# Zoe187419/ATE_replication_causalML

Hardware: AMD Instinct MI355X
Metric: rows/sec for DML-ATE cross-fit, N=1e7 p=500, 1/2/4/8 MI355X; ATE/SE parity (higher is better)
Workload: dtype bf16; 1 GPU; model=DML-PLR 5-fold cross-fit, CV-LASSO nuisances (100 lambdas, inner 4-fold CV), global_batch=10000000, seq_len=500, N=10000000, p=500, folds=5, parallelism=dp1, dgp=tutorial, n_kept=10000000, layout=blocked64+bytes8

## Files before the change

### ate_replication_causalml_amd/_native.py

```python
from __future__ import annotations

import ctypes
import os
from pathlib import Path

_LIBDIR = Path(__file__).resolve().parent / "_lib"
_hip = None
_cpu = None


class NativeMissing(RuntimeError):
    pass


class NativeError(RuntimeError):

    def __init__(self, name: str, status: int, detail: str):
        self.entry, self.status = name, status
        super().__init__(f"{name} failed with status {status}: {detail}")


HIP_ERRORS = {
    1: "hipErrorInvalidValue", 2: "hipErrorOutOfMemory", 3: "hipErrorNotInitialized",
    4: "hipErrorDeinitialized", 9: "hipErrorInvalidConfiguration",
# ... 37 lines not shown
    "ate_chol_solve": "pipiipdpppppp",
    "ate_chol_solve_k": "pipipidppppp",
    "ate_spd_solve_batched": "ppiippp",
    "ate_predict": "ipllppiidipp",
    "ate_irls_update": "ipllppiiiiippppipp",
    "ate_irls_check": "piidippp",
    "ate_naive": "ippplpppp",
    "ate_clip_propensity": "pplpp",
    "ate_aipw": "ppppppldpppp",
    "ate_dml_moments": "ppplppp",
    "ate_dml_finalize": "pipp",
    "ate_boot_multinomial": "ppluiipp",
    "ate_boot_poisson": "ppluiilipp",
    "ate_enet_prepare": "piipipiipipipppppppp",
    "ate_enet_prepare_fused": "piipipiipipi" + "ppppppp" + "plp",
    "ate_enet_path": "pipiippppidddipppppippp",
    "ate_enet_coef": "ppiiiipppppppp",
    "ate_enet_cvloss_gauss": "pippiipppiiipp",
    "ate_cv_select": "pppiipippppip",
    "ate_enet_pick": "ppiiipppip",
    "ate_enet_cv_tail": "pippiipppi" + "pppppp" + "iiii" + "pppppppppppp",
    "ate_dml_resid_moments": "ipllpipipiiiiiippp",
    "ate_dml_resid_moments_final": "ipllpipipiiiiii" + "ppppp",
    "ate_dml_resid_exact": "pllpipipiiiiiiippp",
    "ate_irm_score_moments": "ipllpipiipiiiiidippp",
    "ate_irm_score_moments_multi": "ipllpipiipipiiiiiidippp",
    "ate_irm_score_multi_smax": "",
    "ate_irm_scores": "ipllpipiipiiiiidipp",
    "ate_irm_sens_moments": "ipllpipiipiiiiidippp",
    "ate_irm_target_moments": "ipllpipiipiiiiidippp",
# ... 170 lines not shown
```

### ate_replication_causalml_amd/estimators/lasso.py

```python
from __future__ import annotations

import numpy as np
import torch

from .. import _native
from ..ops import enet as enet_ops
from ..ops import stats as S
from ..ops.devconst import const
from ..ops.enet import cv_enet_gaussian
from ..ops.gram import gram
from ..ops.linalg import chol_solve, chol_solve_active
from ..ops.panel import build_panel, dtype_code
from ..parallel import rng
from ..reference.estimators import lambda_interp
from ..result import AteResult
from ..utils.graphs import estimator_graphs
from .common import as_np, read_result, resolve_device


def _fold_ids(n, K, seed, stream, dist):
    return dist.fold_ids(K, seed, stream) if dist is not None else rng.fold_ids(n, K, seed, stream)


def _sharded_gram(pan, dist):
# ... 306 lines not shown
            return None
        cv = cv_enet_gaussian(st["G"], pan, pan.xcols, ycols,
                              full_sets=[full_sets[k] for k in mine], seg_counts=seg_counts)
        return cv

    def pick(cv):
        return (cv.coef_min if lambda_rule == "min" else cv.coef_1se).reshape(
            len(mine), 2, -1).contiguous()

    fused_final = enet_ops.CV_FUSED and not dist and pan.data.is_cuda

    def phase_fit(st):
        cv = fit(st)
        coef = pick(cv)
        if fused_final:
            mom, res = dml_residual_moments(pan, coef, final=True)
            return {**st, "cv": cv, "mom": mom, "res": res}
        return {**st, "cv": cv, "mom": dml_residual_moments(pan, coef)}

    def phase_fit_sharded(st):
        cv = fit(st)
        coef = torch.zeros((K, 2, p1), dtype=torch.float64, device=pan.device)
        if cv is not None:
            coef.index_copy_(0, const(mine, torch.int64, pan.device), pick(cv).double())
        return {**st, "cv": cv, "coef": coef}

    def phase_resid(st):
        return {**st, "mom": dml_residual_moments(pan, st["coef"])}

    def phase_final(st):
        if "res" in st:
# ... 163 lines not shown
    dev = pan.device
    xc = const(pan.xcols, torch.int32, dev)
    segs = const(np.asarray(pan.seg_bounds[:K], dtype=np.int64), torch.int64, dev)
    nbx = 512
    part = torch.empty(K * nbx * (7 if mode == 1 else 14), dtype=torch.float64, device=dev)
    cs, bs = pan.strides()
    c = coef.double().contiguous()
    _native.call("ate_dml_resid_exact", pan.data.data_ptr(), cs, bs, xc.data_ptr(), len(pan.xcols),
                 segs.data_ptr(), K, c.data_ptr(), pan.cols["Y_hi"], pan.cols["Y_lo"],
                 pan.cols["W_hi"], pan.cols["W_lo"], pan.cols["one"], nbx, mode,
                 None if sh is None else sh.data_ptr(), part.data_ptr(),
                 torch.cuda.current_stream().cuda_stream)
    return part


def dml_residual_moments(pan, coef: torch.Tensor, final: bool = False):
    K = coef.shape[0]
    p = len(pan.xcols)
    if not pan.data.is_cuda:
        X = pan.colmajor().double()
        moms = torch.zeros(7, dtype=torch.float64)
        for k in range(K):
            r0, r1 = pan.seg_bounds[k]
            Xs = X[:, r0:r1]
            v = Xs[pan.cols["one"]] != 0
            xs = Xs[pan.xcols]
            yv, wv = Xs[pan.cols["Y"]], Xs[pan.cols["W"]]
            yr = yv - (coef[k, 0, 0] + coef[k, 0, 1:] @ xs)
            wr = wv - (coef[k, 1, 0] + coef[k, 1, 1:] @ xs)
            moms += S.dml_moments(yr[v], wr[v])
        return moms
    dev = pan.device
    xc = const(pan.xcols, torch.int32, dev)
    segs = const(np.asarray(pan.seg_bounds[:K], dtype=np.int64), torch.int64, dev)
    bf = pan.dtype == torch.bfloat16
    nbx = 512 if bf else 256
    part = torch.empty(K * nbx * 7, dtype=torch.float64, device=dev)
    mom = torch.empty(7, dtype=torch.float64, device=dev)
    bf = pan.dtype == torch.bfloat16
    y0, y1 = (pan.cols["Y_hi"], pan.cols["Y_lo"]) if bf else (pan.cols["Y"], -1)
    w0, w1 = (pan.cols["W_hi"], pan.cols["W_lo"]) if bf else (pan.cols["W"], -1)
    cs, bs = pan.strides()
    if final:
        res = torch.empty(2, dtype=torch.float64, device=dev)
        done = torch.zeros(1, dtype=torch.int32, device=dev)
        _native.call("ate_dml_resid_moments_final", dtype_code(pan.data), pan.data.data_ptr(), cs,
                     bs, xc.data_ptr(), p, segs.data_ptr(), K, coef.data_ptr(), y0, y1, w0, w1,
                     pan.cols["one"], nbx, part.data_ptr(), done.data_ptr(), mom.data_ptr(),
                     res.data_ptr(), torch.cuda.current_stream().cuda_stream)
        return mom, res
    _native.call("ate_dml_resid_moments", dtype_code(pan.data), pan.data.data_ptr(), cs, bs,
                 xc.data_ptr(), p, segs.data_ptr(), K, coef.data_ptr(), y0, y1, w0, w1,
                 pan.cols["one"], nbx, part.data_ptr(), mom.data_ptr(),
                 torch.cuda.current_stream().cuda_stream)
    return mom


def _dml_body(pan, folds, lambda_rule, dist=None, counts=None):
    comm = dist.comm if dist is not None else None
    return dml_crossfit_panel(pan, folds, lambda_rule, comm=comm,
# ... 48 lines not shown
```

### ate_replication_causalml_amd/ops/enet.py

```python
from __future__ import annotations

import os
from dataclasses import dataclass

import numpy as np
import torch

from .. import _native
from ..reference import glmnet as ref
from .devconst import const, const_bytes


def _stream():
    return torch.cuda.current_stream().cuda_stream


CV_FUSED = os.environ.get("ATE_CV_FUSED", "1") not in ("", "0")


@dataclass
class EnetCvResult:
    lambdas: torch.Tensor
    nlam: torch.Tensor
    cvm: torch.Tensor
    cvsd: torch.Tensor
    sel: torch.Tensor
    coef_path: torch.Tensor
    coef_min: torch.Tensor
    coef_1se: torch.Tensor
    full_keys: list
    npass: torch.Tensor
    fold_npass: torch.Tensor | None = None
    fold_nlam: torch.Tensor | None = None

    def check(self):
        bad = [] if self.fold_npass is None else \
            np.flatnonzero(self.fold_npass.cpu().numpy() < 0).tolist()
        if bad:
            from ..utils.guards import NumericalError
            raise NumericalError(f"CV fold path(s) {bad} timed out waiting for their "
                                 "full-data lambda sequence; selection is invalid")
        return self


def poison_if_truncated(fold_npass: torch.Tensor, *ts):
    bad = (fold_npass < 0).any()
    nan = torch.full((), float("nan"), dtype=torch.float64, device=fold_npass.device)
    return [torch.where(bad, nan, t) for t in ts]


def _zeroed(dev, *specs):
    sizes = [int(np.prod(sh)) * torch.empty((), dtype=dt).element_size() for sh, dt in specs]
    offs = np.concatenate([[0], np.cumsum([(b + 255) // 256 * 256 for b in sizes])])
    buf = torch.zeros(int(offs[-1]), dtype=torch.uint8, device=dev)
    return [buf[int(o):int(o) + b].view(dt).view(sh)
            for (sh, dt), o, b in zip(specs, offs[:-1], sizes)]


def _rescale_vp(vp, p):
    vp = np.ones(p) if vp is None else np.maximum(np.asarray(vp, float), 0)
    return vp * p / vp.sum()


def _cv_tables(nseg, full_sets, ycols, nreal, nlambda, full_y):
    ny = len(ycols)
    if full_sets is None:
        full_sets = [list(range(nseg))]
    tsets, tindex = [], {}

    def tid(segs):
        key = tuple(sorted(segs))
# ... 97 lines not shown
    nt = masks.shape[0]
    masks_t = const(masks, torch.uint8, dev)
    xc = const(xcols, torch.int32, dev)
    yc = const(ycols, torch.int32, dev)
    c_f32 = int(panel_dtype != torch.float64)
    ldc = (p + 63) // 64 * 64
    nf = len(full_probs)
    probs_all = list(full_probs) + list(fold_probs)
    nq = len(probs_all)
    i32 = torch.int32
    c_dt = torch.float32 if c_f32 else torch.float64
    fused = CV_FUSED and L <= 256
    fused_prep = fused and nseg <= 8
    if fused:
        zspec = [((nq, L), torch.float64), ((nq,), i32), ((nq,), i32), ((nq,), i32), ((nf,), i32)]
        if not fused_prep:
            zspec.append(((nt, p, ldc), c_dt))
        rsq, nlam, npass, progress, done, *zc = _zeroed(dev, *zspec)
        C = zc[0] if zc else torch.empty((nt, p, ldc), dtype=c_dt, device=dev)
        apath = torch.empty((nq, L, p), **f64)
    else:
        C, apath, rsq, nlam, npass, progress = _zeroed(
            dev, ((nt, p, ldc), c_dt), ((nq, L, p), torch.float64),
            ((nq, L), torch.float64), ((nq,), i32), ((nq,), i32), ((nq,), i32))
    g = torch.empty((nt, ny, p), **f64)
    xm = torch.empty((nt, p), **f64)
    xs = torch.empty((nt, p), **f64)
    ju = torch.empty((nt, p), dtype=torch.uint8, device=dev)
    ym = torch.empty((nt, ny), **f64)
    ys = torch.empty((nt, ny), **f64)
    nobs = torch.empty(nt, **f64)
    if fused_prep:
        lams = torch.empty((nq, L), **f64)
        _native.call("ate_enet_prepare_fused", G.data_ptr(), nseg, P, masks_t.data_ptr(), nt,
                     xc.data_ptr(), p, one, yc.data_ptr(), ny, C.data_ptr(), c_f32, g.data_ptr(),
                     xm.data_ptr(), xs.data_ptr(), ju.data_ptr(), ym.data_ptr(), ys.data_ptr(),
                     nobs.data_ptr(), lams.data_ptr(), nq * L, s)
    else:
        _native.call("ate_enet_prepare", G.data_ptr(), nseg, P, masks_t.data_ptr(), nt,
                     xc.data_ptr(), p, one, yc.data_ptr(), ny, C.data_ptr(), c_f32, g.data_ptr(),
                     xm.data_ptr(), xs.data_ptr(), ju.data_ptr(), ym.data_ptr(), ys.data_ptr(),
                     nobs.data_ptr(), s)
        lams = torch.full((nq, L), float("nan"), **f64)
    vp_t = const(np.asarray(vp, dtype=np.float64), torch.float64, dev)
    pr = _probs_tensor(probs_all, dev)
    lampub = torch.empty((nq, L), **f64)
    _native.call("ate_enet_path", C.data_ptr(), c_f32, g.data_ptr(), p, ny, ju.data_ptr(),
                 ys.data_ptr(), vp_t.data_ptr(), pr.data_ptr(), nq, alpha, flmin, thresh,
                 maxit, apath.data_ptr(), lams.data_ptr(), rsq.data_ptr(), nlam.data_ptr(),
                 npass.data_ptr(), L, progress.data_ptr(), lampub.data_ptr(), s)
    hold = const([0] * nf + list(fold_holds), torch.int32, dev)
    ycol_p = const([0] * nf + list(fold_ycol), torch.int32, dev)
# ... 4 lines not shown
    cvsd = torch.empty((nf, L), **f64)
    sel = torch.empty((nf, 2), dtype=torch.int32, device=dev)
    K = fold_index.shape[1]
    cmin = torch.empty((nf, p + 1), **f64)
    c1se = torch.empty((nf, p + 1), **f64)
    fold_npass = npass[nf:]
    if fused:
        coef = torch.empty((nf, L, p + 1), **f64)
        _native.call("ate_enet_cv_tail", G.data_ptr(), P, hold.data_ptr(), xc.data_ptr(), p, one,
                     ycol_p.data_ptr(), apath.data_ptr(), pr.data_ptr(), ny, nlam.data_ptr(),
                     xm.data_ptr(), xs.data_ptr(), ju.data_ptr(), ym.data_ptr(), ys.data_ptr(), L,
                     nf, nq - nf, K, fidx.data_ptr(), nfold_t.data_ptr(), coef.data_ptr(),
                     cvraw.data_ptr(), cvm.data_ptr(), cvsd.data_ptr(), sel.data_ptr(),
                     cmin.data_ptr(), c1se.data_ptr(), fold_npass.data_ptr(), done.data_ptr(), s)
        return EnetCvResult(lams[:nf], nlam[:nf], cvm, cvsd, sel, coef, cmin, c1se, full_keys,
                            npass[:nf], fold_npass, nlam[nf:])
    coef = torch.empty((nq, L, p + 1), **f64)
    _native.call("ate_enet_coef", apath.data_ptr(), pr.data_ptr(), nq, p, ny, L,
                 nlam.data_ptr(), xm.data_ptr(), xs.data_ptr(), ju.data_ptr(), ym.data_ptr(),
                 ys.data_ptr(), coef.data_ptr(), s)
    _native.call("ate_enet_cvloss_gauss", G.data_ptr(), P, hold.data_ptr(), xc.data_ptr(), p, one,
                 ycol_p.data_ptr(), coef.data_ptr(), nlam.data_ptr(), L, nf, nq - nf,
                 cvraw.data_ptr(), s)
    _native.call("ate_cv_select", cvraw.data_ptr(), fidx.data_ptr(), nfold_t.data_ptr(), K, nf,
                 nlam.data_ptr(), L, cvm.data_ptr(), cvsd.data_ptr(), sel.data_ptr(),
                 fold_npass.data_ptr(), nq - nf, s)
    _native.call("ate_enet_pick", coef.data_ptr(), sel.data_ptr(), p, L, nf, cmin.data_ptr(),
                 c1se.data_ptr(), fold_npass.data_ptr(), nq - nf, s)
    return EnetCvResult(lams[:nf], nlam[:nf], cvm, cvsd, sel, coef[:nf], cmin, c1se, full_keys,
                        npass[:nf], fold_npass, nlam[nf:])

# ... 79 lines not shown
```

### csrc/enet.hip

```cpp
#include <cstdlib>

#include <utility>

#include "common.hpp"

#include <type_traits>

using namespace ate;

__device__ __forceinline__ double seg_sum(const double* __restrict__ G, int nseg, int P,
                                          const unsigned char* __restrict__ mk, int a, int b) {
  double acc = 0.0;
  for (int q = 0; q < nseg; ++q)
    if (mk[q]) acc += G[((int64_t)q * P + a) * P + b];
  return acc;
}

__device__ __forceinline__ void col_mean_var(double s1, double s2, double n, double& m,
                                             double& v) {
  m = s1 / n;
  v = s2 / n - m * m;
}
__device__ __forceinline__ double std_entry(double sab, double n, double ma, double mb,
                                            double sa, double sb) {
// ... 106 lines not shown
  for (int q = 0; q < PF_SEG; ++q) v[q] = q < nseg ? G[((int64_t)q * P + a) * P + b] : 0.0;
  double acc = 0.0;
#pragma unroll
  for (int q = 0; q < PF_SEG; ++q)
    if (q < nseg && (bits >> q & 1u)) acc += v[q];
  return acc;
}

template <typename CT>
__global__ __launch_bounds__(256) void enet_prepare_fused_kernel(
    const double* __restrict__ G, int nseg, int P, const unsigned char* __restrict__ masks,
    int ntrain, const int* __restrict__ xcols, int p, int ldc, int ones_col,
    const int* __restrict__ ycols, int ny, CT* __restrict__ C, double* __restrict__ g,
    double* __restrict__ xm, double* __restrict__ xs, unsigned char* __restrict__ ju,
    double* __restrict__ ym, double* __restrict__ ys, double* __restrict__ nobs,
    double* __restrict__ lams, int64_t nlams) {
  const int tk = blockIdx.x, tj = blockIdx.y, tid = threadIdx.x;
  const int j0 = tj * PF_TJ, k0 = tk * PF_TK, s0 = blockIdx.z * PF_SCH;
  const int lane = tid & 63, jr = tid >> 6;
  ATE_DASSERT(k0 + PF_TK <= ldc && j0 < p && ones_col >= 0 && ones_col < P);
  {
    const int64_t nb = (int64_t)gridDim.x * gridDim.y * gridDim.z,
                  b = ((int64_t)blockIdx.z * gridDim.y + tj) * gridDim.x + tk;
    for (int64_t e = b * 256 + tid; e < nlams; e += nb * 256) lams[e] = __builtin_nan("");
  }
  __shared__ double s_n[PF_SCH], s_m[PF_SCH][PF_NC], s_s[PF_SCH][PF_NC];
  __shared__ unsigned char s_ju[PF_SCH][PF_NC];
  __shared__ unsigned s_mask[PF_SCH];
  const bool inreg = nseg <= PF_SEG;
  const int k = k0 + lane;
  const int xk = k < p ? xcols[k] : 0;
  ATE_DASSERT(xk >= 0 && xk < P);
  double gv[4][PF_SEG];
  int xj[4];
#pragma unroll
  for (int i = 0; i < 4; ++i) {
    const int j = j0 + jr + 4 * i;
    xj[i] = j < p ? xcols[j] : 0;
    ATE_DASSERT(xj[i] >= 0 && xj[i] < P);
// ... 87 lines not shown
        double gj = 0.0;
        if (s_ju[sl][jl]) {
          const int yc = ycols[y];
          ATE_DASSERT(yc >= 0 && yc < P);
          double my, vy;
          col_mean_var(set_sum(s, sl, ones_col, yc), set_sum(s, sl, yc, yc), s_n[sl], my, vy);
          gj = std_entry(set_sum(s, sl, xcols[j], yc), s_n[sl], s_m[sl][jl], my, s_s[sl][jl],
                         vy > 0 ? sqrt(vy) : 1.0);
        }
        g[((int64_t)s * ny + y) * p + j] = gj;
      }
    }
  }
}

ATE_API int ate_enet_prepare_fused(const void* G, int nseg, int P, const void* masks, int ntrain,
                                   const void* xcols, int p, int ones_col, const void* ycols,
                                   int ny, void* C, int c_f32, void* g, void* xm, void* xs,
                                   void* ju, void* ym, void* ys, void* nobs, void* lams,
                                   int64_t nlams, void* stream) {
  if (p < 1 || ntrain < 1 || nseg < 1 || ny < 0) return -1;
  hipStream_t st = (hipStream_t)stream;
  const int ldc = (p + 63) / 64 * 64;
  dim3 grid(ldc / PF_TK, (p + PF_TJ - 1) / PF_TJ, (ntrain + PF_SCH - 1) / PF_SCH);
  if (c_f32)
    ATE_LAUNCH(enet_prepare_fused_kernel<float>, grid, dim3(256), 0, st, (const double*)G, nseg,
               P, (const unsigned char*)masks, ntrain, (const int*)xcols, p, ldc, ones_col,
               (const int*)ycols, ny, (float*)C, (double*)g, (double*)xm, (double*)xs,
               (unsigned char*)ju, (double*)ym, (double*)ys, (double*)nobs, (double*)lams, nlams);
  else
    ATE_LAUNCH(enet_prepare_fused_kernel<double>, grid, dim3(256), 0, st, (const double*)G, nseg,
               P, (const unsigned char*)masks, ntrain, (const int*)xcols, p, ldc, ones_col,
               (const int*)ycols, ny, (double*)C, (double*)g, (double*)xm, (double*)xs,
               (unsigned char*)ju, (double*)ym, (double*)ys, (double*)nobs, (double*)lams, nlams);
  ATE_CHECK_LAUNCH();
  return 0;
}

struct EnetProblem {
  int train;
  int y;
  int ulam_src;
  int nlam_req;
};

constexpr double BIGL = 9.9e35;
constexpr int PMAX = 512;

#ifdef ENET_PROF
__device__ unsigned long long enet_prof[256][32];
#define PROF_T(var) const unsigned long long var = wall_clock64()
#define PROF_ADD(k, v) do { if (tid == 0) sprof[0][k] += (unsigned long long)(v); } while (0)
#else
#define PROF_T(var)
#define PROF_ADD(k, v) do { } while (0)
#endif

template <typename CT> struct VecT;
template <> struct VecT<float> { typedef float4 type; };
template <> struct VecT<double> { typedef double2 type; };
__device__ __forceinline__ float vdot(float4 a, float4 b) {
  return a.x * b.x + a.y * b.y + a.z * b.z + a.w * b.w;
}
__device__ __forceinline__ double vdot(double2 a, double2 b) { return a.x * b.x + a.y * b.y; }

// ... 61 lines not shown
#define ENET_S_ENTER 40
#endif
#ifndef ENET_S_FETCH
#define ENET_S_FETCH 8
#endif
constexpr int S_UNION = 112 * 1024;
constexpr int S_CAP = S_UNION / (PMAX * 4);
#ifndef ENET_DENSE_MIN
#define ENET_DENSE_MIN 28
#endif

#define LDS_AS __attribute__((address_space(3)))
struct PassS {
  double dlx, rsq;
};
__device__ __noinline__ PassS enet_pass_s(bool full, int T, int ldc, double ab, double dem,
                                          const float* __restrict__ Cf, LDS_AS double* sg,
                                          LDS_AS double* sa, const LDS_AS double* svp,
                                          LDS_AS int* sflag, LDS_AS int* sslot,
                                          LDS_AS float* sccache, LDS_AS int* sever_n,
                                          LDS_AS int* sncache,
                                          LDS_AS unsigned long long* sprof_row) {
  const int lane = threadIdx.x & 63;
#ifdef ENET_PROF
  const long long tps0_ = clock64();
  unsigned long long nit_ = 0, nfetch_ = 0;
#endif
  double gS[8], aS[8], tS[8];
  int slS[8];
  int flb = 0;
#pragma unroll
  for (int s8 = 0; s8 < 8; ++s8) {
    const int k = s8 * 64 + lane;
    const bool in = s8 < T;
    gS[s8] = in ? sg[k] : 0.0;
    aS[s8] = in ? sa[k] : 0.0;
    tS[s8] = in ? svp[k] * ab : 0.0;
    slS[s8] = in ? sslot[k] : -1;
    const int f = in ? sflag[k] : 0;
    if ((f & 1) && (full || (f & 2))) flb |= 1 << s8;
    if (f & 2) flb |= 1 << (8 + s8);
  }
  int ncache = __builtin_amdgcn_readfirstlane(*sncache);
  int ever_n = __builtin_amdgcn_readfirstlane(*sever_n);
  double dlx = 0.0, rsq_add = 0.0;
#ifdef ENET_PROF
  const long long tpl0_ = clock64();
#endif
  static_for<8>([&](auto s_tag) __attribute__((always_inline)) {
    constexpr int SJ = decltype(s_tag)::value;
    if (SJ >= T) return;
    uint64_t live = ~0ull;
    for (;;) {
      const bool c = ((flb >> SJ) & 1) & ((aS[SJ] != 0.0) | (fabs(gS[SJ] + aS[SJ]) > tS[SJ]));
      const uint64_t cm = __builtin_amdgcn_ballot_w64(c) & live;
      if (!cm) break;
      const int lj = __ffsll((unsigned long long)cm) - 1;
      live = lj == 63 ? 0ull : (~0ull << (lj + 1));
#ifdef ENET_PROF
      ++nit_;
#endif
      const int j = SJ * 64 + lj;
      const double gj = readlane_d(gS[SJ], lj);
      const double aj = readlane_d(aS[SJ], lj);
      const double tj = readlane_d(tS[SJ], lj);
      int slj = __builtin_amdgcn_readlane(slS[SJ], lj);
      const double uj = gj + aj;
      double an = copysign(fmax(fabs(uj) - tj, 0.0), uj);
      if (dem != 0.0) an = an / (1.0 + svp[j] * dem);
      const double d = an - aj;
      if (__builtin_amdgcn_readfirstlane((int)(d == 0.0))) continue;
      float cv[8];
      if (slj < 0 && ncache < S_CAP) {
#ifdef ENET_PROF
        ++nfetch_;
#endif
        slj = ncache++;
        const float* Cj = Cf + (int64_t)j * ldc;
        LDS_AS float* dst = sccache + slj * PMAX;
#pragma unroll
        for (int s8 = 0; s8 < 8; ++s8) {
          const int k = s8 * 64 + lane;
          const float v = k < ldc ? Cj[k] : 0.f;
          cv[s8] = v;
          dst[(s8 >> 2) * 256 + lane * 4 + (s8 & 3)] = v;
        }
        if (lane == 0) sslot[j] = slj;
        if (lane == lj) slS[SJ] = slj;
      } else if (slj >= 0) {
        const LDS_AS float* src = sccache + slj * PMAX + lane * 4;
#pragma unroll
        for (int e = 0; e < 4; ++e) {
          cv[e] = src[e];
          cv[4 + e] = src[256 + e];
        }
      } else {
        const float* Cj = Cf + (int64_t)j * ldc;
#pragma unroll
        for (int s8 = 0; s8 < 8; ++s8) cv[s8] = s8 * 64 + lane < ldc ? Cj[s8 * 64 + lane] : 0.f;
      }
#pragma unroll
      for (int s8 = 0; s8 < 8; ++s8) gS[s8] = __builtin_fma(-(double)cv[s8], d, gS[s8]);
      const int evj = __builtin_amdgcn_readlane(flb, lj);
      if (!((evj >> (8 + SJ)) & 1)) ++ever_n;
      if (lane == lj) {
        flb |= 1 << (8 + SJ);
        aS[SJ] = an;
      }
      rsq_add += d * (2.0 * gj - d);
      dlx = fmax(dlx, d * d);
    }
  });
#ifdef ENET_PROF
  if (lane == 0) sprof_row[23] += (unsigned long long)(clock64() - tpl0_);
#endif
#pragma unroll
  for (int s8 = 0; s8 < 8; ++s8) {
    if (s8 < T) {
      const int k = s8 * 64 + lane;
      sg[k] = gS[s8];
      sa[k] = aS[s8];
      if ((flb >> (8 + s8)) & 1) sflag[k] |= 2;
    }
  }
  if (lane == 0) {
    *sever_n = ever_n;
    *sncache = ncache;
  }
#ifdef ENET_PROF
  if (lane == 0) {
    sprof_row[19] += 1ull;
    sprof_row[20] += nit_;
    sprof_row[21] += (unsigned long long)(clock64() - tps0_);
    sprof_row[22] += nfetch_;
  }
#endif
  return PassS{dlx, rsq_add};
}

constexpr int FOLD_LEAD = 2;

__device__ __noinline__ double lambda0_extrap(double l1, double l2) {
#pragma clang fp contract(off)
  return exp(2.0 * log(l1) - log(l2));
}

template <typename CT, bool LASSO>
__global__ __launch_bounds__(NTH) void enet_path_kernel(
    const CT* __restrict__ C, const double* __restrict__ gin, int p, int ny,
    const unsigned char* __restrict__ ju_s, const double* __restrict__ ys_s,
    const double* __restrict__ vp_in, const EnetProblem* __restrict__ probs, int nprob,
    double alpha, double flmin, double thr, int maxit,
    double* __restrict__ apath, double* __restrict__ lams, double* __restrict__ rsqs,
    int* __restrict__ nlam_out, int* __restrict__ npass_out, int L, int* __restrict__ progress,
    long spin_max, double* __restrict__ lampub) {
  constexpr int TMAX = PMAX / 64;
  __shared__ double sg[PMAX], sa[PMAX], svp[PMAX], sdc[PMAX];
  __shared__ __attribute__((aligned(16))) unsigned char s_union[S_UNION];
  double(&sds)[TMAX][PMAX] = *reinterpret_cast<double(*)[TMAX][PMAX]>(s_union);
  float(&sCn2)[2][64 * 64] = *reinterpret_cast<float(*)[2][64 * 64]>(s_union + 32768);
  float(&sCorr)[64 * 64] = *reinterpret_cast<float(*)[64 * 64]>(s_union + 65536);
  float* const sccache = reinterpret_cast<float*>(s_union);
  __shared__ int sslot[PMAX];
  __shared__ int sever_n;
  __shared__ int sncache;
  __shared__ int spub, sarr;
  __shared__ int sfetch0;
  __shared__ int sflag[PMAX];
  __shared__ double spart2[2][NW][64];
  __shared__ __attribute__((aligned(16))) float sred[NW][256];
  __shared__ __attribute__((aligned(16))) float sdw[NW][64];
  __shared__ int srow[NW][64];
  __shared__ float scorr2[2][NP][64];
  __shared__ int scorr_ok[2];
#ifdef ENET_PROF
  __shared__ unsigned long long sprof[NW][32];
  for (int e = threadIdx.x; e < NW * 32; e += blockDim.x) (&sprof[0][0])[e] = 0ull;
#endif
  __shared__ __attribute__((aligned(16))) CT sdelta[PMAX];
  __shared__ int slist[PMAX];
  constexpr int PER = (PMAX + NP - 1) / NP + 1;
  __shared__ int slist2[NP * PER];
  __shared__ __attribute__((aligned(16))) CT sdelta2[NP * PER];
  __shared__ int scl[64];
  __shared__ CT scd[64];
  __shared__ __attribute__((aligned(16))) float sdall[64];
  __shared__ int svis[8], snv, sblk_any[8], svis_id[8];
  __shared__ double sdl;
  __shared__ double srsq;
  __shared__ int snl_final;
  __shared__ int sany;
  __shared__ int schg;
// ... 18 lines not shown
  for (int k = tid; k < T * 64; k += NTH) {
    bool in = k < p;
    sg[k] = in ? gin[((int64_t)pr.train * ny + pr.y) * p + k] : 0.0;
    sa[k] = 0.0;
    svp[k] = in ? vp_in[k] : 0.0;
    sdc[k] = 0.0;
    sflag[k] = (in && ju_s[(int64_t)pr.train * p + k]) ? 1 : 0;
  }
  for (int e = tid; e < TMAX * PMAX; e += NTH) (&sds[0][0])[e] = 0.0;
  for (int k = tid; k < PMAX; k += NTH) sslot[k] = -1;
  if (tid < 8) svis_id[tid] = tid;
  if (tid == 0) { sever_n = 0; sncache = 0; spub = 0; sarr = 0; sfetch0 = 0; }
  __syncthreads();
  const int nlam = pr.ulam_src >= 0 ? L : pr.nlam_req;
  const double alf = pr.ulam_src >= 0 ? 1.0 : pow(flmin, 1.0 / (double)(nlam - 1));
  double alm = 0.0, rsq = 0.0, rsq_prev = 0.0;
  int npass = 0, m_out = 0;
  double ab = 0.0, dem = 0.0;
  double rsq_l = 0.0;
  typedef typename VecT<CT>::type V;
  constexpr int W = sizeof(V) / sizeof(CT);
  float dg_lo[32], dg_hi[32];
  int cpar = 0;

  auto pull_block = [&](int jb, int tb) __attribute__((always_inline)) -> float {
    ATE_DASSERT(jb >= 0 && jb < T && tb >= 0 && tb < T && jb != tb);
    const int grp = lane >> 4, c4 = (lane & 15) * 4;
    const int j = jb * 64 + lane;
    const double ddj = sdc[j] - sds[tb][j];
    const uint64_t nzb = __builtin_amdgcn_ballot_w64(ddj != 0.0);
// ... 225 lines not shown
        const PassS r = enet_pass_s(
            full, T, ldc, ab, dem, reinterpret_cast<const float*>(Cq), (LDS_AS double*)sg,
            (LDS_AS double*)sa, (const LDS_AS double*)svp, (LDS_AS int*)sflag,
            (LDS_AS int*)sslot, (LDS_AS float*)sccache, (LDS_AS int*)&sever_n,
            (LDS_AS int*)&sncache,
#ifdef ENET_PROF
            (LDS_AS unsigned long long*)&sprof[0][0]
#else
            nullptr
#endif
        );
        if (lane == 0) {
          sdl = r.dlx;
          rsq_l += r.rsq;
        }
      }
      __syncthreads();
      const double r = sdl;
      __syncthreads();
      return r;
    }
    double dlx_l = 0.0;
    int nv = T;
    if (!full) {
      for (int t = wid; t < T; t += NW) {
        const bool a = (sflag[t * 64 + lane] & 3) == 3;
        const uint64_t b = __builtin_amdgcn_ballot_w64(a);
        if (lane == 0) sblk_any[t] = b != 0;
      }
      __syncthreads();
// ... 431 lines not shown
        double x = alm, x2 = alm;
        lp[1] = x * ysq;
        for (int mm = 2; mm < L; ++mm) {
          x *= alf;
          lp[mm] = x * ysq;
          if (mm == 2) x2 = x;
        }
        lp[0] = lambda0_extrap(lp[1], x2 * ysq);
        publish(2);
      }
    } else {
      alm *= alf;
    }
    ab = alm * alpha;
    dem = LASSO ? 0.0 : alm * (1.0 - alpha);
    const int fetched = sncache - sfetch0;
    __syncthreads();
    if (tid == 0) sfetch0 = sncache;
    if (modeS && (sever_n > ENET_S_ENTER || fetched > ENET_S_FETCH)) {
      modeS = false;
      for (int e = tid; e < TMAX * PMAX; e += NTH) (&sds[0][0])[e] = 0.0;
      ready = -1;
      __syncthreads();
    }
#ifdef ENET_PROF
    const unsigned long long tpass0_ = wall_clock64();
    if (tid == 0) sprof[0][29] += tpass0_ - tlam0_;
#endif
    while (npass < maxit) {
      ++npass;
      double dl = pass(true);
      if (dl < thr) break;
      while (npass < maxit) {
// ... 51 lines not shown
      ATE_DASSERT(m_out - nl <= FOLD_LEAD + 1);
      for (int mm = nl; mm < m_out; ++mm) {
        double* ap = apath + ((int64_t)q * L + mm) * p;
        for (int k = tid; k < p; k += NTH) ap[k] = 0.0;
        if (tid == 0) {
          lams[(int64_t)q * L + mm] = __builtin_nan("");
          rsqs[(int64_t)q * L + mm] = 0.0;
        }
      }
      npass = nl > 0 ? snpass_ring[(nl - 1) & 3] : 0;
      m_out = nl;
    }
  }
#ifdef ENET_PROF
  __syncthreads();
  if (tid < 32) {
    unsigned long long acc = 0;
    for (int w = 0; w < NW; ++w) acc += sprof[w][tid];
    if (tid == 10) acc = (unsigned long long)(clock64() - kc0_);
    if (tid == 11) acc = wall_clock64() - kw0_;
    atomicAdd(&enet_prof[q][tid], acc);
  }
#endif
  if (tid == 0) {
    nlam_out[q] = m_out;
    npass_out[q] = timed_out ? -1 : npass;
    if (!is_fold) publish(1 << 30);
  }
}

#ifdef ENET_PROF
extern "C" __attribute__((visibility("default"))) int ate_enet_prof_read(void* host) {
  return (int)hipMemcpyFromSymbol(host, HIP_SYMBOL(enet_prof), sizeof(enet_prof));
}
extern "C" __attribute__((visibility("default"))) int ate_enet_prof_reset() {
  static unsigned long long z[256][32];
  return (int)hipMemcpyToSymbol(HIP_SYMBOL(enet_prof), z, sizeof(z));
}
#endif

ATE_KERNEL_SHAPE("enet_path_kernel<float, lasso>", NTH, 0, enet_path_kernel<float, true>)
ATE_KERNEL_SHAPE("enet_path_kernel<float, enet>", NTH, 0, enet_path_kernel<float, false>)
ATE_KERNEL_SHAPE("enet_path_kernel<double, lasso>", NTH, 0, enet_path_kernel<double, true>)
ATE_KERNEL_SHAPE("enet_path_kernel<double, enet>", NTH, 0, enet_path_kernel<double, false>)

ATE_API int ate_enet_path(const void* C, int c_f32, const void* g, int p, int ny, const void* ju,
                          const void* ys, const void* vp, const void* probs, int nprob,
                          double alpha, double flmin, double thr, int maxit, void* apath,
                          void* lams, void* rsqs, void* nlam_out, void* npass_out, int L,
                          void* progress, void* lampub, void* stream) {
  if (p > PMAX) return -2;
  if (nprob > 256) return -3;
  hipStream_t s = (hipStream_t)stream;
  const int nwg = (nprob + 7) / 8 * 8;
  const char* sm = getenv("ATE_ENET_SPIN_MAX");
  const long spin_max = sm ? atol(sm) : (1l << 26);
#define LAUNCH_C(CTT, LS)                                                                      \
  ATE_LAUNCH((enet_path_kernel<CTT, LS>), dim3(nwg), dim3(NTH), 0, s, (const CTT*)C,   \
                     (const double*)g, p, ny, (const unsigned char*)ju, (const double*)ys,     \
                     (const double*)vp, (const EnetProblem*)probs, nprob, alpha, flmin, thr,   \
                     maxit, (double*)apath, (double*)lams, (double*)rsqs, (int*)nlam_out,     \
                     (int*)npass_out, L, (int*)progress, spin_max, (double*)lampub)
  const bool lasso = alpha == 1.0;
  if (c_f32 && lasso) LAUNCH_C(float, true);
  else if (c_f32) LAUNCH_C(float, false);
  else if (lasso) LAUNCH_C(double, true);
  else LAUNCH_C(double, false);
#undef LAUNCH_C
  ATE_CHECK_LAUNCH();
  return 0;
}

template <class Store>
__device__ __forceinline__ double coef_row_terms(const double* __restrict__ a, int64_t tb, int p,
                                                 double ysq, const double* __restrict__ xm,
                                                 const double* __restrict__ xs,
                                                 const unsigned char* __restrict__ ju, int t0,
// ... 444 lines not shown
```

Measured before the change: 2.272 billion rows/s.

## Prefetch likely-entering LASSO columns into LDS cache with idle waves; fold zeroing into prepare

In the coordinate-descent path kernel's sparse mode, waves that would otherwise sit idle now speculatively load Gram columns for features likely to enter at the next lambda (strong-rule style screening) into the LDS column cache. Cache slots are claimed atomically, so the pass code reads slot state with atomics and fences. Separately, the per-call zero-initialised counters and done flags are cleared inside the fused prepare kernel rather than by a separate memset, and a spare zeroed word is reused as the final moments 'done' flag, removing small allocation and zeroing launches. The prefetch adds atomic and fence overhead and can spend cache slots on columns that never enter.

New measurement: 2.325 billion rows/s (median of 6 runs). 1.02x the previous value.

```diff
diff --git a/ate_replication_causalml_amd/_native.py b/ate_replication_causalml_amd/_native.py
--- a/ate_replication_causalml_amd/_native.py
+++ b/ate_replication_causalml_amd/_native.py
@@ -75,6 +75,7 @@
     "ate_boot_poisson": "ppluiilipp",
     "ate_enet_prepare": "piipipiipipipppppppp",
     "ate_enet_prepare_fused": "piipipiipipi" + "ppppppp" + "plp",
+    "ate_enet_prepare_fused_clear": "piipipiipipi" + "ppppppp" + "pl" + "pl" + "p",
     "ate_enet_path": "pipiippppidddipppppippp",
     "ate_enet_coef": "ppiiiipppppppp",
     "ate_enet_cvloss_gauss": "pippiipppiiipp",
diff --git a/ate_replication_causalml_amd/estimators/lasso.py b/ate_replication_causalml_amd/estimators/lasso.py
--- a/ate_replication_causalml_amd/estimators/lasso.py
+++ b/ate_replication_causalml_amd/estimators/lasso.py
@@ -344,7 +344,7 @@
         cv = fit(st)
         coef = pick(cv)
         if fused_final:
-            mom, res = dml_residual_moments(pan, coef, final=True)
+            mom, res = dml_residual_moments(pan, coef, final=True, done=cv.spare_zero)
             return {**st, "cv": cv, "mom": mom, "res": res}
         return {**st, "cv": cv, "mom": dml_residual_moments(pan, coef)}
 
@@ -538,7 +538,7 @@
     return part
 
 
-def dml_residual_moments(pan, coef: torch.Tensor, final: bool = False):
+def dml_residual_moments(pan, coef: torch.Tensor, final: bool = False, done=None):
     K = coef.shape[0]
     p = len(pan.xcols)
     if not pan.data.is_cuda:
@@ -567,7 +567,8 @@
     cs, bs = pan.strides()
     if final:
         res = torch.empty(2, dtype=torch.float64, device=dev)
-        done = torch.zeros(1, dtype=torch.int32, device=dev)
+        if done is None:
+            done = torch.zeros(1, dtype=torch.int32, device=dev)
         _native.call("ate_dml_resid_moments_final", dtype_code(pan.data), pan.data.data_ptr(), cs,
                      bs, xc.data_ptr(), p, segs.data_ptr(), K, coef.data_ptr(), y0, y1, w0, w1,
                      pan.cols["one"], nbx, part.data_ptr(), done.data_ptr(), mom.data_ptr(),
diff --git a/ate_replication_causalml_amd/ops/enet.py b/ate_replication_causalml_amd/ops/enet.py
--- a/ate_replication_causalml_amd/ops/enet.py
+++ b/ate_replication_causalml_amd/ops/enet.py
@@ -32,6 +32,7 @@
     npass: torch.Tensor
     fold_npass: torch.Tensor | None = None
     fold_nlam: torch.Tensor | None = None
+    spare_zero: torch.Tensor | None = None
 
     def check(self):
         bad = [] if self.fold_npass is None else \
@@ -55,6 +56,14 @@
     buf = torch.zeros(int(offs[-1]), dtype=torch.uint8, device=dev)
     return [buf[int(o):int(o) + b].view(dt).view(sh)
             for (sh, dt), o, b in zip(specs, offs[:-1], sizes)]
+
+
+def _carved(dev, *specs):
+    sizes = [int(np.prod(sh)) * torch.empty((), dtype=dt).element_size() for sh, dt in specs]
+    offs = np.concatenate([[0], np.cumsum([(b + 255) // 256 * 256 for b in sizes])])
+    buf = torch.empty(int(offs[-1]), dtype=torch.uint8, device=dev)
+    return buf, [buf[int(o):int(o) + b].view(dt).view(sh)
+                 for (sh, dt), o, b in zip(specs, offs[:-1], sizes)]
 
 
 def _rescale_vp(vp, p):
@@ -182,10 +191,13 @@
     fused_prep = fused and nseg <= 8
     if fused:
         zspec = [((nq, L), torch.float64), ((nq,), i32), ((nq,), i32), ((nq,), i32), ((nf,), i32)]
-        if not fused_prep:
+        spare = zbuf = None
+        if fused_prep:
+            zbuf, (rsq, nlam, npass, progress, done, spare) = _carved(dev, *zspec, ((1,), i32))
+            C = torch.empty((nt, p, ldc), dtype=c_dt, device=dev)
+        else:
             zspec.append(((nt, p, ldc), c_dt))
-        rsq, nlam, npass, progress, done, *zc = _zeroed(dev, *zspec)
-        C = zc[0] if zc else torch.empty((nt, p, ldc), dtype=c_dt, device=dev)
+            rsq, nlam, npass, progress, done, C = _zeroed(dev, *zspec)
         apath = torch.empty((nq, L, p), **f64)
     else:
         C, apath, rsq, nlam, npass, progress = _zeroed(
@@ -200,10 +212,11 @@
     nobs = torch.empty(nt, **f64)
     if fused_prep:
         lams = torch.empty((nq, L), **f64)
-        _native.call("ate_enet_prepare_fused", G.data_ptr(), nseg, P, masks_t.data_ptr(), nt,
-                     xc.data_ptr(), p, one, yc.data_ptr(), ny, C.data_ptr(), c_f32, g.data_ptr(),
-                     xm.data_ptr(), xs.data_ptr(), ju.data_ptr(), ym.data_ptr(), ys.data_ptr(),
-                     nobs.data_ptr(), lams.data_ptr(), nq * L, s)
+        _native.call("ate_enet_prepare_fused_clear", G.data_ptr(), nseg, P, masks_t.data_ptr(),
+                     nt, xc.data_ptr(), p, one, yc.data_ptr(), ny, C.data_ptr(), c_f32,
+                     g.data_ptr(), xm.data_ptr(), xs.data_ptr(), ju.data_ptr(), ym.data_ptr(),
+                     ys.data_ptr(), nobs.data_ptr(), lams.data_ptr(), nq * L, zbuf.data_ptr(),
+                     zbuf.numel() // 4, s)
     else:
         _native.call("ate_enet_prepare", G.data_ptr(), nseg, P, masks_t.data_ptr(), nt,
                      xc.data_ptr(), p, one, yc.data_ptr(), ny, C.data_ptr(), c_f32, g.data_ptr(),
@@ -238,7 +251,7 @@
                      cvraw.data_ptr(), cvm.data_ptr(), cvsd.data_ptr(), sel.data_ptr(),
                      cmin.data_ptr(), c1se.data_ptr(), fold_npass.data_ptr(), done.data_ptr(), s)
         return EnetCvResult(lams[:nf], nlam[:nf], cvm, cvsd, sel, coef, cmin, c1se, full_keys,
-                            npass[:nf], fold_npass, nlam[nf:])
+                            npass[:nf], fold_npass, nlam[nf:], spare)
     coef = torch.empty((nq, L, p + 1), **f64)
     _native.call("ate_enet_coef", apath.data_ptr(), pr.data_ptr(), nq, p, ny, L,
                  nlam.data_ptr(), xm.data_ptr(), xs.data_ptr(), ju.data_ptr(), ym.data_ptr(),
diff --git a/csrc/enet.hip b/csrc/enet.hip
--- a/csrc/enet.hip
+++ b/csrc/enet.hip
@@ -144,7 +144,7 @@
     const int* __restrict__ ycols, int ny, CT* __restrict__ C, double* __restrict__ g,
     double* __restrict__ xm, double* __restrict__ xs, unsigned char* __restrict__ ju,
     double* __restrict__ ym, double* __restrict__ ys, double* __restrict__ nobs,
-    double* __restrict__ lams, int64_t nlams) {
+    double* __restrict__ lams, int64_t nlams, unsigned* __restrict__ zero, int64_t nzero) {
   const int tk = blockIdx.x, tj = blockIdx.y, tid = threadIdx.x;
   const int j0 = tj * PF_TJ, k0 = tk * PF_TK, s0 = blockIdx.z * PF_SCH;
   const int lane = tid & 63, jr = tid >> 6;
@@ -153,6 +153,7 @@
     const int64_t nb = (int64_t)gridDim.x * gridDim.y * gridDim.z,
                   b = ((int64_t)blockIdx.z * gridDim.y + tj) * gridDim.x + tk;
     for (int64_t e = b * 256 + tid; e < nlams; e += nb * 256) lams[e] = __builtin_nan("");
+    for (int64_t e = b * 256 + tid; e < nzero; e += nb * 256) zero[e] = 0u;
   }
   __shared__ double s_n[PF_SCH], s_m[PF_SCH][PF_NC], s_s[PF_SCH][PF_NC];
   __shared__ unsigned char s_ju[PF_SCH][PF_NC];
@@ -270,12 +271,12 @@
   }
 }
 
-ATE_API int ate_enet_prepare_fused(const void* G, int nseg, int P, const void* masks, int ntrain,
-                                   const void* xcols, int p, int ones_col, const void* ycols,
-                                   int ny, void* C, int c_f32, void* g, void* xm, void* xs,
-                                   void* ju, void* ym, void* ys, void* nobs, void* lams,
-                                   int64_t nlams, void* stream) {
-  if (p < 1 || ntrain < 1 || nseg < 1 || ny < 0) return -1;
+static int enet_prepare_fused_launch(const void* G, int nseg, int P, const void* masks, int ntrain,
+                                     const void* xcols, int p, int ones_col, const void* ycols,
+                                     int ny, void* C, int c_f32, void* g, void* xm, void* xs,
+                                     void* ju, void* ym, void* ys, void* nobs, void* lams,
+                                     int64_t nlams, void* zero, int64_t nzero, void* stream) {
+  if (p < 1 || ntrain < 1 || nseg < 1 || ny < 0 || nzero < 0 || (nzero > 0 && !zero)) return -1;
   hipStream_t st = (hipStream_t)stream;
   const int ldc = (p + 63) / 64 * 64;
   dim3 grid(ldc / PF_TK, (p + PF_TJ - 1) / PF_TJ, (ntrain + PF_SCH - 1) / PF_SCH);
@@ -283,14 +284,37 @@
     ATE_LAUNCH(enet_prepare_fused_kernel<float>, grid, dim3(256), 0, st, (const double*)G, nseg,
                P, (const unsigned char*)masks, ntrain, (const int*)xcols, p, ldc, ones_col,
                (const int*)ycols, ny, (float*)C, (double*)g, (double*)xm, (double*)xs,
-               (unsigned char*)ju, (double*)ym, (double*)ys, (double*)nobs, (double*)lams, nlams);
+               (unsigned char*)ju, (double*)ym, (double*)ys, (double*)nobs, (double*)lams, nlams,
+               (unsigned*)zero, nzero);
   else
     ATE_LAUNCH(enet_prepare_fused_kernel<double>, grid, dim3(256), 0, st, (const double*)G, nseg,
                P, (const unsigned char*)masks, ntrain, (const int*)xcols, p, ldc, ones_col,
                (const int*)ycols, ny, (double*)C, (double*)g, (double*)xm, (double*)xs,
-               (unsigned char*)ju, (double*)ym, (double*)ys, (double*)nobs, (double*)lams, nlams);
+               (unsigned char*)ju, (double*)ym, (double*)ys, (double*)nobs, (double*)lams, nlams,
+               (unsigned*)zero, nzero);
   ATE_CHECK_LAUNCH();
   return 0;
+}
+
+ATE_API int ate_enet_prepare_fused(const void* G, int nseg, int P, const void* masks, int ntrain,
+                                   const void* xcols, int p, int ones_col, const void* ycols,
+                                   int ny, void* C, int c_f32, void* g, void* xm, void* xs,
+                                   void* ju, void* ym, void* ys, void* nobs, void* lams,
+                                   int64_t nlams, void* stream) {
+  return enet_prepare_fused_launch(G, nseg, P, masks, ntrain, xcols, p, ones_col, ycols, ny, C,
+                                   c_f32, g, xm, xs, ju, ym, ys, nobs, lams, nlams, nullptr, 0,
+                                   stream);
+}
+
+ATE_API int ate_enet_prepare_fused_clear(const void* G, int nseg, int P, const void* masks,
+                                         int ntrain, const void* xcols, int p, int ones_col,
+                                         const void* ycols, int ny, void* C, int c_f32, void* g,
+                                         void* xm, void* xs, void* ju, void* ym, void* ys,
+                                         void* nobs, void* lams, int64_t nlams, void* zero,
+                                         int64_t nzero, void* stream) {
+  return enet_prepare_fused_launch(G, nseg, P, masks, ntrain, xcols, p, ones_col, ycols, ny, C,
+                                   c_f32, g, xm, xs, ju, ym, ys, nobs, lams, nlams, zero, nzero,
+                                   stream);
 }
 
 struct EnetProblem {
@@ -304,7 +328,8 @@
 constexpr int PMAX = 512;
 
 #ifdef ENET_PROF
-__device__ unsigned long long enet_prof[256][32];
+constexpr int PROF_N = 40;
+__device__ unsigned long long enet_prof[256][PROF_N];
 #define PROF_T(var) const unsigned long long var = wall_clock64()
 #define PROF_ADD(k, v) do { if (tid == 0) sprof[0][k] += (unsigned long long)(v); } while (0)
 #else
@@ -396,6 +421,91 @@
 struct PassS {
   double dlx, rsq;
 };
+constexpr int SLOT_NONE = -1, SLOT_FLIGHT = -2;
+constexpr int S_SPEC = S_CAP - ENET_S_ENTER - 1;
+static_assert(S_SPEC >= 0, "mode S: the column cache holds every mover below the switch point");
+
+__device__ __forceinline__ int enet_take_slot(LDS_AS int* sncache, int limit) {
+  int slot = -1;
+  if ((threadIdx.x & 63) == 0) {
+    int cur = __hip_atomic_load(sncache, __ATOMIC_RELAXED, __HIP_MEMORY_SCOPE_WORKGROUP);
+    while (cur < limit) {
+      if (__hip_atomic_compare_exchange_strong(sncache, &cur, cur + 1, __ATOMIC_RELAXED,
+                                               __ATOMIC_RELAXED, __HIP_MEMORY_SCOPE_WORKGROUP)) {
+        slot = cur;
+        break;
+      }
+    }
+  }
+  return __builtin_amdgcn_readfirstlane(slot);
+}
+
+__device__ __forceinline__ int enet_take_slot_w0(LDS_AS int* sncache) {
+  int got = S_CAP;
+  if (__builtin_amdgcn_readfirstlane(__hip_atomic_load(
+          sncache, __ATOMIC_RELAXED, __HIP_MEMORY_SCOPE_WORKGROUP)) < S_CAP) {
+    if ((threadIdx.x & 63) == 0)
+      got = __hip_atomic_fetch_add(sncache, 1, __ATOMIC_RELAXED, __HIP_MEMORY_SCOPE_WORKGROUP);
+    got = __builtin_amdgcn_readfirstlane(got);
+  }
+  return got;
+}
+
+__device__ __noinline__ void enet_prefetch_s(int hw, int T, int ldc, double abr,
+                                             const float* __restrict__ Cf,
+                                             const LDS_AS double* sg, const LDS_AS double* sa,
+                                             const LDS_AS double* svp, const LDS_AS int* sflag,
+                                             LDS_AS int* sslot, LDS_AS float* sccache,
+                                             const LDS_AS int* sever_n, LDS_AS int* sncache,
+                                             LDS_AS unsigned long long* sprof_row) {
+  const int lane = threadIdx.x & 63;
+  const int limit = min(S_CAP, min(*sever_n, S_CAP) + S_SPEC);
+  for (int s = hw; s < T; s += NP) {
+    const int k = s * 64 + lane;
+    const bool hit = (sflag[k] & 1) && sslot[k] == SLOT_NONE && sa[k] == 0.0 &&
+                     fabs(sg[k]) > svp[k] * abr;
+    uint64_t hm = __builtin_amdgcn_ballot_w64(hit);
+    while (hm) {
+      if (__builtin_amdgcn_readfirstlane(__hip_atomic_load(
+              sncache, __ATOMIC_RELAXED, __HIP_MEMORY_SCOPE_WORKGROUP)) >= limit)
+        return;
+      const int lj = __ffsll((unsigned long long)hm) - 1;
+      hm &= hm - 1;
+      const int j = s * 64 + lj;
+      int claimed = 0;
+      if (lane == 0) {
+        int expect = SLOT_NONE;
+        claimed = __hip_atomic_compare_exchange_strong(sslot + j, &expect, SLOT_FLIGHT,
+                                                       __ATOMIC_RELAXED, __ATOMIC_RELAXED,
+                                                       __HIP_MEMORY_SCOPE_WORKGROUP);
+      }
+      if (!__builtin_amdgcn_readfirstlane(claimed)) continue;
+      const int slot = enet_take_slot(sncache, limit);
+      if (slot < 0) {
+        if (lane == 0) {
+          int expect = SLOT_FLIGHT;
+          __hip_atomic_compare_exchange_strong(sslot + j, &expect, SLOT_NONE, __ATOMIC_RELAXED,
+                                               __ATOMIC_RELAXED, __HIP_MEMORY_SCOPE_WORKGROUP);
+        }
+        return;
+      }
+      ATE_DASSERT(slot < S_CAP && j < T * 64);
+      const float* Cj = Cf + j * ldc;
+      float v[8];
+#pragma unroll
+      for (int s8 = 0; s8 < 8; ++s8) v[s8] = Cj[min(s8, T - 1) * 64 + lane];
+      LDS_AS float* dst = sccache + slot * PMAX;
+#pragma unroll
+      for (int s8 = 0; s8 < 8; ++s8) dst[(s8 >> 2) * 256 + lane * 4 + (s8 & 3)] = v[s8];
+      __builtin_amdgcn_fence(__ATOMIC_RELEASE, "workgroup");
+      if (lane == 0)
+        __hip_atomic_store(sslot + j, slot, __ATOMIC_RELAXED, __HIP_MEMORY_SCOPE_WORKGROUP);
+#ifdef ENET_PROF
+      if (lane == 0) sprof_row[32] += 1ull;
+#endif
+    }
+  }
+}
 __device__ __noinline__ PassS enet_pass_s(bool full, int T, int ldc, double ab, double dem,
                                           const float* __restrict__ Cf, LDS_AS double* sg,
                                           LDS_AS double* sa, const LDS_AS double* svp,
@@ -406,7 +516,7 @@
   const int lane = threadIdx.x & 63;
 #ifdef ENET_PROF
   const long long tps0_ = clock64();
-  unsigned long long nit_ = 0, nfetch_ = 0;
+  unsigned long long nit_ = 0, nfetch_ = 0, nused_ = 0;
 #endif
   double gS[8], aS[8], tS[8];
   int slS[8];
@@ -423,7 +533,6 @@
     if ((f & 1) && (full || (f & 2))) flb |= 1 << s8;
     if (f & 2) flb |= 1 << (8 + s8);
   }
-  int ncache = __builtin_amdgcn_readfirstlane(*sncache);
   int ever_n = __builtin_amdgcn_readfirstlane(*sever_n);
   double dlx = 0.0, rsq_add = 0.0;
 #ifdef ENET_PROF
@@ -453,22 +562,36 @@
       const double d = an - aj;
       if (__builtin_amdgcn_readfirstlane((int)(d == 0.0))) continue;
       float cv[8];
-      if (slj < 0 && ncache < S_CAP) {
-#ifdef ENET_PROF
-        ++nfetch_;
-#endif
-        slj = ncache++;
-        const float* Cj = Cf + (int64_t)j * ldc;
+#ifdef ENET_PROF
+      int own_ = slj < 0;
+#endif
+      if (slj < 0) {
+        slj = __builtin_amdgcn_readfirstlane(__hip_atomic_load(
+            sslot + j, __ATOMIC_RELAXED, __HIP_MEMORY_SCOPE_WORKGROUP));
+        __builtin_amdgcn_fence(__ATOMIC_ACQUIRE, "workgroup");
+        if (slj >= 0 && lane == lj) slS[SJ] = slj;
+#ifdef ENET_PROF
+        own_ = slj < 0;
+#endif
+      }
+      int got;
+      if (slj == SLOT_NONE && (got = enet_take_slot_w0(sncache)) < S_CAP) {
+        slj = got;
+        const float* Cj = Cf + j * ldc;
         LDS_AS float* dst = sccache + slj * PMAX;
 #pragma unroll
         for (int s8 = 0; s8 < 8; ++s8) {
           const int k = s8 * 64 + lane;
-          const float v = k < ldc ? Cj[k] : 0.f;
+          const float v = Cj[min(s8, T - 1) * 64 + lane];
           cv[s8] = v;
           dst[(s8 >> 2) * 256 + lane * 4 + (s8 & 3)] = v;
         }
-        if (lane == 0) sslot[j] = slj;
+        if (lane == 0)
+          __hip_atomic_store(sslot + j, slj, __ATOMIC_RELAXED, __HIP_MEMORY_SCOPE_WORKGROUP);
         if (lane == lj) slS[SJ] = slj;
+#ifdef ENET_PROF
+        own_ = 1;
+#endif
       } else if (slj >= 0) {
         const LDS_AS float* src = sccache + slj * PMAX + lane * 4;
 #pragma unroll
@@ -477,14 +600,20 @@
           cv[4 + e] = src[256 + e];
         }
       } else {
-        const float* Cj = Cf + (int64_t)j * ldc;
-#pragma unroll
-        for (int s8 = 0; s8 < 8; ++s8) cv[s8] = s8 * 64 + lane < ldc ? Cj[s8 * 64 + lane] : 0.f;
+        ATE_DASSERT(slj == SLOT_FLIGHT || ever_n > ENET_S_ENTER);
+        const float* Cj = Cf + j * ldc;
+#pragma unroll
+        for (int s8 = 0; s8 < 8; ++s8) cv[s8] = Cj[min(s8, T - 1) * 64 + lane];
       }
 #pragma unroll
       for (int s8 = 0; s8 < 8; ++s8) gS[s8] = __builtin_fma(-(double)cv[s8], d, gS[s8]);
       const int evj = __builtin_amdgcn_readlane(flb, lj);
-      if (!((evj >> (8 + SJ)) & 1)) ++ever_n;
+      if (!((evj >> (8 + SJ)) & 1)) {
+        ++ever_n;
+#ifdef ENET_PROF
+        if (own_) ++nfetch_; else ++nused_;
+#endif
+      }
       if (lane == lj) {
         flb |= 1 << (8 + SJ);
         aS[SJ] = an;
@@ -505,16 +634,14 @@
       if ((flb >> (8 + s8)) & 1) sflag[k] |= 2;
     }
   }
-  if (lane == 0) {
-    *sever_n = ever_n;
-    *sncache = ncache;
-  }
+  if (lane == 0) *sever_n = ever_n;
 #ifdef ENET_PROF
   if (lane == 0) {
     sprof_row[19] += 1ull;
     sprof_row[20] += nit_;
     sprof_row[21] += (unsigned long long)(clock64() - tps0_);
     sprof_row[22] += nfetch_;
+    sprof_row[33] += nused_;
   }
 #endif
   return PassS{dlx, rsq_add};
@@ -535,7 +662,7 @@
     double alpha, double flmin, double thr, int maxit,
     double* __restrict__ apath, double* __restrict__ lams, double* __restrict__ rsqs,
     int* __restrict__ nlam_out, int* __restrict__ npass_out, int L, int* __restrict__ progress,
-    long spin_max, double* __restrict__ lampub) {
+    long spin_max, double* __restrict__ lampub, int s_prefetch) {
   constexpr int TMAX = PMAX / 64;
   __shared__ double sg[PMAX], sa[PMAX], svp[PMAX], sdc[PMAX];
   __shared__ __attribute__((aligned(16))) unsigned char s_union[S_UNION];
@@ -556,8 +683,8 @@
   __shared__ float scorr2[2][NP][64];
   __shared__ int scorr_ok[2];
 #ifdef ENET_PROF
-  __shared__ unsigned long long sprof[NW][32];
-  for (int e = threadIdx.x; e < NW * 32; e += blockDim.x) (&sprof[0][0])[e] = 0ull;
+  __shared__ unsigned long long sprof[NW][PROF_N];
+  for (int e = threadIdx.x; e < NW * PROF_N; e += blockDim.x) (&sprof[0][0])[e] = 0ull;
 #endif
   __shared__ __attribute__((aligned(16))) CT sdelta[PMAX];
   __shared__ int slist[PMAX];
@@ -606,6 +733,7 @@
   __syncthreads();
   const int nlam = pr.ulam_src >= 0 ? L : pr.nlam_req;
   const double alf = pr.ulam_src >= 0 ? 1.0 : pow(flmin, 1.0 / (double)(nlam - 1));
+  const double lam_ratio = pr.ulam_src < 0 ? alf : L > 1 ? pow(flmin, 1.0 / (double)(L - 1)) : 1.0;
   double alm = 0.0, rsq = 0.0, rsq_prev = 0.0;
   int npass = 0, m_out = 0;
   double ab = 0.0, dem = 0.0;
@@ -861,6 +989,18 @@
           sdl = r.dlx;
           rsq_l += r.rsq;
         }
+      } else if (s_prefetch) {
+        enet_prefetch_s(wid - 1, T, ldc, ab * lam_ratio, reinterpret_cast<const float*>(Cq),
+                        (const LDS_AS double*)sg, (const LDS_AS double*)sa,
+                        (const LDS_AS double*)svp, (const LDS_AS int*)sflag, (LDS_AS int*)sslot,
+                        (LDS_AS float*)sccache, (const LDS_AS int*)&sever_n,
+                        (LDS_AS int*)&sncache,
+#ifdef ENET_PROF
+                        (LDS_AS unsigned long long*)&sprof[wid][0]
+#else
+                        nullptr
+#endif
+        );
       }
       __syncthreads();
       const double r = sdl;
@@ -1322,9 +1462,10 @@
     }
     ab = alm * alpha;
     dem = LASSO ? 0.0 : alm * (1.0 - alpha);
-    const int fetched = sncache - sfetch0;
+    const int evc = min(sever_n, S_CAP);
+    const int fetched = evc - sfetch0;
     __syncthreads();
-    if (tid == 0) sfetch0 = sncache;
+    if (tid == 0) sfetch0 = evc;
     if (modeS && (sever_n > ENET_S_ENTER || fetched > ENET_S_FETCH)) {
       modeS = false;
       for (int e = tid; e < TMAX * PMAX; e += NTH) (&sds[0][0])[e] = 0.0;
@@ -1406,7 +1547,7 @@
   }
 #ifdef ENET_PROF
   __syncthreads();
-  if (tid < 32) {
+  if (tid < PROF_N) {
     unsigned long long acc = 0;
     for (int w = 0; w < NW; ++w) acc += sprof[w][tid];
     if (tid == 10) acc = (unsigned long long)(clock64() - kc0_);
@@ -1426,7 +1567,7 @@
   return (int)hipMemcpyFromSymbol(host, HIP_SYMBOL(enet_prof), sizeof(enet_prof));
 }
 extern "C" __attribute__((visibility("default"))) int ate_enet_prof_reset() {
-  static unsigned long long z[256][32];
+  static unsigned long long z[256][PROF_N];
   return (int)hipMemcpyToSymbol(HIP_SYMBOL(enet_prof), z, sizeof(z));
 }
 #endif
@@ -1447,12 +1588,14 @@
   const int nwg = (nprob + 7) / 8 * 8;
   const char* sm = getenv("ATE_ENET_SPIN_MAX");
   const long spin_max = sm ? atol(sm) : (1l << 26);
+  const char* sp = getenv("ATE_ENET_S_PREFETCH");
+  const int s_prefetch = sp ? atoi(sp) != 0 : 1;
 #define LAUNCH_C(CTT, LS)                                                                      \
   ATE_LAUNCH((enet_path_kernel<CTT, LS>), dim3(nwg), dim3(NTH), 0, s, (const CTT*)C,   \
                      (const double*)g, p, ny, (const unsigned char*)ju, (const double*)ys,     \
                      (const double*)vp, (const EnetProblem*)probs, nprob, alpha, flmin, thr,   \
                      maxit, (double*)apath, (double*)lams, (double*)rsqs, (int*)nlam_out,     \
-                     (int*)npass_out, L, (int*)progress, spin_max, (double*)lampub)
+                     (int*)npass_out, L, (int*)progress, spin_max, (double*)lampub, s_prefetch)
   const bool lasso = alpha == 1.0;
   if (c_f32 && lasso) LAUNCH_C(float, true);
   else if (c_f32) LAUNCH_C(float, false);
```
